# BassyKuo/DAVO

Measured on NVIDIA B200. Metric: PoseNN+attention frame-pairs/sec @128x416, higher is better.
Workload: dtype tf32 operands (activations and weights), fp32 accumulate; inputs read as given (uint8 frames, float32 flow and labels; flow_f16 off)

## Files before the change

davo_b200/_capi.py:

```python
from __future__ import annotations

import ctypes as C
import os

from . import build as _build

_LIB = None

SYMBOLS = (
    "davo_create", "davo_set_weight", "davo_finalize_weights", "davo_forward",
    "davo_forward_host", "davo_get_intermediate", "davo_last_launch_count",
    "davo_last_host_copy_bytes",
    "davo_profile_layers", "davo_debug_set_conv_impl", "davo_forward_pairs", "davo_forward_host_pairs",
    "davo_forward_features", "davo_debug_flows_to_half", "davo_debug_labels_to_bytes", "davo_forward_host_compact", "davo_bind_host_numa",
    "davo_compose_trajectory", "davo_kitti_errors", "davo_decode_jpeg_batch",
    "davo_forward_host_pairs_async", "davo_forward_host_compact_async", "davo_host_wait",
    "davo_comm_unique_id", "davo_comm_create", "davo_comm_world", "davo_allgather_poses",
    "davo_forward_sequence", "davo_forward_sequence_host",
    "davo_odometry_create", "davo_odometry_push", "davo_odometry_reset", "davo_odometry_frames",
    "davo_odometry_push_many", "davo_odometry_push_many_host", "davo_odometry_move",
    "davo_last_error",
    "davo_destroy", "davo_build_info", "davo_config_bytes", "davo_odometry_destroy",
)


class DavoConfigC(C.Structure):
    _fields_ = [(n, C.c_int32) for n in (
        "H", "W", "max_batch", "posenn", "cnv6_out", "in_mode", "att_src", "att_tgt_ones",
        "mask_mode", "se_act", "flow_abs", "flow_norm", "posenn_se", "micro_batch", "depth_norm", "se_pool", "se_hidden",
        "pixel_map", "depth_split", "flow_f16", "batch_norm")]


class DavoFeaturesC(C.Structure):
    _fields_ = [(n, C.c_void_p) for n in (
        "image", "attention", "masked_image", "seg_19", "seg_color", "flow_color", "cnv6_rot", "cnv6_trans")]


def lib_path() -> str:
    return _build.LIB


def load() -> C.CDLL:
    global _LIB
    if _LIB is not None:
        return _LIB
    path = lib_path()
    if _build.is_stale():
        try:
            _build.build()
        except Exception as e:
            if not os.path.exists(path):
                raise ImportError("libdavo_b200.so is not built and cannot be built here: %s" % e)
    try:
        lib = C.CDLL(path)
    except OSError as e:
        raise ImportError("cannot load %s: %s (there is no CPU fallback)" % (path, e))
    for s in SYMBOLS:
        if not hasattr(lib, s):
            raise ImportError("%s does not export %s" % (path, s))
    vp, ip, fp = C.c_void_p, C.c_int, C.POINTER(C.c_float)
    lib.davo_create.argtypes = [C.POINTER(DavoConfigC), ip, C.POINTER(vp)]
    lib.davo_set_weight.argtypes = [vp, C.c_char_p, vp, C.POINTER(C.c_int64), ip]
    lib.davo_finalize_weights.argtypes = [vp]
    lib.davo_forward.argtypes = [vp, ip, vp, vp, vp, vp, vp, vp]
    lib.davo_forward_host.argtypes = [vp, ip, vp, vp, vp, vp, vp, vp]
    lib.davo_forward_pairs.argtypes = [vp, ip, ip, vp, vp, vp, vp, vp, vp]
    lib.davo_forward_host_pairs.argtypes = [vp, ip, ip, vp, vp, vp, vp, vp, vp]
    lib.davo_forward_host_compact.argtypes = [vp, ip, ip, vp, vp, vp, vp, vp, vp]
    lib.davo_bind_host_numa.argtypes = [vp]
    lib.davo_compose_trajectory.argtypes = [vp, vp, ip, vp, vp]
    lib.davo_kitti_errors.argtypes = [vp, vp, vp, ip, vp, fp, vp]
    lib.davo_decode_jpeg_batch.argtypes = [vp, C.POINTER(vp), C.POINTER(C.c_int64), ip, vp, vp]
    lib.davo_forward_host_pairs_async.argtypes = [vp, ip, ip, vp, vp, vp, vp, vp, vp, C.POINTER(C.c_longlong)]
    lib.davo_forward_host_compact_async.argtypes = [vp, ip, ip, vp, vp, vp, vp, vp, vp, C.POINTER(C.c_longlong)]
    lib.davo_host_wait.argtypes = [vp, C.c_longlong]
    lib.davo_forward_sequence.argtypes = [vp, ip, ip, vp, vp, vp, vp, vp, vp, vp]
    lib.davo_forward_sequence_host.argtypes = [vp, ip, ip, vp, vp, vp, vp, vp, vp, vp, C.POINTER(C.c_longlong)]
    lib.davo_odometry_create.argtypes = [vp, ip, ip, ip, C.POINTER(vp)]
    lib.davo_odometry_push.argtypes = [vp, ip, vp, vp, vp, vp, vp, vp, vp, C.POINTER(ip), C.POINTER(ip), vp,
                                       C.POINTER(C.c_longlong)]
    lib.davo_odometry_push_many.argtypes = [ip, C.POINTER(vp), C.POINTER(ip)] + [C.POINTER(vp)] * 7 + [
        C.POINTER(ip), C.POINTER(ip), vp]
    lib.davo_odometry_push_many_host.argtypes = [ip, C.POINTER(vp), C.POINTER(ip)] + [C.POINTER(vp)] * 7 + [
        C.POINTER(ip), C.POINTER(ip), vp, C.POINTER(C.c_longlong)]
    lib.davo_odometry_move.argtypes = [vp, vp]
    lib.davo_odometry_reset.argtypes = [vp]
    lib.davo_odometry_frames.argtypes = [vp, C.POINTER(C.c_longlong), C.POINTER(C.c_longlong)]
    lib.davo_odometry_destroy.argtypes = [vp]
    lib.davo_odometry_destroy.restype = None
    lib.davo_get_intermediate.argtypes = [vp, C.c_char_p, ip, vp, C.c_int64, C.POINTER(C.c_int64)]
    lib.davo_last_launch_count.argtypes = [vp]
    lib.davo_last_host_copy_bytes.argtypes = [vp, C.POINTER(C.c_longlong), C.POINTER(C.c_longlong)]
    lib.davo_profile_layers.argtypes = [vp, ip, fp, C.POINTER(ip), vp]
    lib.davo_debug_set_conv_impl.argtypes = [vp, ip]
    lib.davo_forward_features.argtypes = [vp, ip, vp, vp, vp, vp, vp, C.POINTER(DavoFeaturesC), vp]
    lib.davo_debug_flows_to_half.argtypes = [vp, vp, C.c_longlong, ip]
    lib.davo_debug_labels_to_bytes.argtypes = [vp, vp, C.c_longlong, ip]
    lib.davo_comm_unique_id.argtypes = [vp]
    lib.davo_comm_create.argtypes = [vp, vp, ip, ip]
    lib.davo_comm_world.argtypes = [vp, C.POINTER(ip), C.POINTER(ip)]
    lib.davo_allgather_poses.argtypes = [vp, vp, vp, ip, vp, vp]
    lib.davo_last_error.argtypes = [vp]
    lib.davo_last_error.restype = C.c_char_p
    lib.davo_destroy.argtypes = [vp]
    lib.davo_destroy.restype = None
    lib.davo_build_info.restype = C.c_char_p
    lib.davo_config_bytes.restype = ip
    if lib.davo_config_bytes() != C.sizeof(DavoConfigC):
        raise ImportError("%s: davo_config is %d bytes in the library, %d in this binding (rebuild: python davo_b200/build.py --force)"
                          % (path, lib.davo_config_bytes(), C.sizeof(DavoConfigC)))
    for s in SYMBOLS[:SYMBOLS.index("davo_last_error")]:
        getattr(lib, s).restype = ip
    _LIB = lib
    return lib


PAIRS = {"all": 0, "trajectory": 1, "trajectory_first": 2}


def last_error(lib, handle) -> str:
    msg = lib.davo_last_error(handle)
    return msg.decode() if msg else ""
```

davo_b200/csrc/conv_cm.cuh:

```cuda
#pragma once
#include "conv_common.cuh"

namespace davo {
namespace cm {

constexpr int kBlockM = 128;
constexpr int kThreads = 352;
constexpr int kEpiWarps = 8;
constexpr int kWBytes = kBlockM * kSlabBytes;

struct ConvParams {
  int num_tiles;
  int num_pixel_tiles;
  int tiles_w, tiles_h, groups, m_blocks;
  int Hout, Wout;
  int out_stride;
  int cout_g;
  int cin_group_off;
  int n_patches, n_taps;
  int patch_w;
  int patch_bytes;
  int patch_stage_bytes;
  int p_stages, w_stages;
  int raw;
  float* out;
  const float* bias;
  float* sum_out;
  PatchDesc patches[kMaxPatches];
  TapDesc taps[kMaxTaps];
};

struct TileCoord { int n, g, mb, h0, w0, t; };

template <int NPIX>
__device__ __forceinline__ TileCoord decode_item_cluster(const ConvParams& p, int item, int rank) {
  TileCoord c;
  c.mb = item % p.m_blocks;
  int r = item / p.m_blocks;
  c.g = r % p.groups;
  const int pp = r / p.groups;
  const int tpi = p.tiles_h * p.tiles_w;
  const int pix = min(2 * pp + rank, p.num_pixel_tiles - 1);
  c.t = pix % tpi;
  c.n = pix / tpi;
  c.h0 = (c.t / p.tiles_w) * (NPIX / kTileW);
  c.w0 = (c.t % p.tiles_w) * kTileW;
  return c;
}

template <int NPIX>
__device__ __forceinline__ TileCoord decode_tile(const ConvParams& p, int tile) {
  TileCoord c;
  c.mb = tile % p.m_blocks;
  int r = tile / p.m_blocks;
  const int tpi = p.tiles_h * p.tiles_w;
  c.t = r % tpi;
  r /= tpi;
  c.g = r % p.groups;
  c.n = r / p.groups;
  c.h0 = (c.t / p.tiles_w) * (NPIX / kTileW);
  c.w0 = (c.t % p.tiles_w) * kTileW;
  return c;
}

template <int NPIX, int EPI, bool STAGED = false, bool CLUSTER = false>
__global__ void __launch_bounds__(kThreads, 1)
conv_tc_kernel(const __grid_constant__ CUtensorMap tmX, const __grid_constant__ CUtensorMap tmW,
               const __grid_constant__ CUtensorMap tmO, const __grid_constant__ ConvParams p) {
  extern __shared__ uint8_t smem_raw[];
  uint8_t* smem = reinterpret_cast<uint8_t*>((reinterpret_cast<uintptr_t>(smem_raw) + 1023) &
                                             ~uintptr_t(1023));
  const int PS = p.p_stages, WS = p.w_stages;
  uint8_t* smem_p = smem;
  uint8_t* smem_w = smem + PS * p.patch_stage_bytes;
  uint8_t* epi_stage = smem_w + WS * kWBytes;
  uint64_t* bars = reinterpret_cast<uint64_t*>(epi_stage + (STAGED ? kEpiWarps * 4096 : 0));
  uint64_t* p_full = bars;
  uint64_t* p_empty = bars + kMaxStages;
  uint64_t* w_full = bars + 2 * kMaxStages;
  uint64_t* w_empty = bars + 3 * kMaxStages;
  uint64_t* acc_full = bars + 4 * kMaxStages;
  uint64_t* acc_empty = acc_full + 2;
  uint32_t* tmem_slot = reinterpret_cast<uint32_t*>(acc_empty + 2);
// ... 23 lines not shown
      mbar_init(&w_empty[i], CLUSTER ? 2 : 1);
    }
    for (int i = 0; i < 2; ++i) {
      mbar_init(&acc_full[i], 1);
      mbar_init(&acc_empty[i], EPI == EPI_STORE_RELU ? kEpiWarps : 4);
    }
    fence_mbar_init();
  }
  if (warp == 1) tmem_alloc(tmem_slot, kTmemCols);
  tc_fence_before();
  __syncthreads();
  if constexpr (CLUSTER) cluster_sync();
  tc_fence_after();
  const uint32_t tmem_base = *tmem_slot;

  if (warp == 0) {
    if (lane == 0) {
      pdl_wait();
      int ps = 0;
      uint32_t pphase = 0;
      for (int tile = first; tile < p.num_tiles; tile += step) {
        const TileCoord tc = decode(tile);
        for (int pi = 0; pi < p.n_patches; ++pi) {
          const PatchDesc d = p.patches[pi];
          TWAIT(0, mbar_wait(&p_empty[ps], pphase ^ 1));
          mbar_expect_tx(&p_full[ps], p.patch_bytes);
          tma_load_5d(smem_p + ps * p.patch_stage_bytes, &tmX, &p_full[ps],
                      tc.g * p.cin_group_off + d.c, tc.w0 + d.dw, d.par, tc.h0 + d.dh, tc.n);
          if (++ps == PS) { ps = 0; pphase ^= 1; }
        }
      }
    }
  } else if (warp == 6) {
    if (lane == 0) {
      int ws = 0;
      uint32_t wphase = 0;
      for (int tile = first; tile < p.num_tiles; tile += step) {
        const TileCoord tc = decode(tile);
        const int row0 = (tc.g * p.m_blocks + tc.mb) * p.n_taps;
        for (int t = 0; t < p.n_taps; ++t) {
          TWAIT(1, mbar_wait(&w_empty[ws], wphase ^ 1));
          mbar_expect_tx(&w_full[ws], kWBytes);
          if constexpr (CLUSTER)
            tma_load_2d_multicast(smem_w + ws * kWBytes + rank * (kWBytes / 2), &tmW, &w_full[ws], 0,
                                  (row0 + p.taps[t].b_idx) * kBlockM + rank * (kBlockM / 2), (uint16_t)3);
          else
            tma_load_2d(smem_w + ws * kWBytes, &tmW, &w_full[ws], 0, (row0 + p.taps[t].b_idx) * kBlockM);
          if (++ws == WS) { ws = 0; wphase ^= 1; }
        }
      }
    }
  } else if (warp == 1) {
    {
      constexpr uint32_t idesc = umma_idesc_tf32(kBlockM, NPIX);
      const uint32_t tmem_u = __shfl_sync(0xffffffffu, tmem_base, 0);
      const uint32_t w_hi = umma_desc_hi(1024), x_hi = umma_desc_hi((uint32_t)p.patch_w * kSlabBytes);
      const uint32_t p_lo0 = umma_desc_lo(smem_u32(smem_p)), p_lo_step = (uint32_t)p.patch_stage_bytes >> 4;
      const uint32_t w_lo0 = umma_desc_lo(smem_u32(smem_w));
      int ps = 0, ws = 0;
      uint32_t pphase = 0, wphase = 0;
      int it = 0;
      for (int tile = first; tile < p.num_tiles; tile += step, ++it) {
        const int acc = it & 1;
        const uint32_t acc_phase = (it >> 1) & 1;
        TWAIT(4, mbar_wait(&acc_empty[acc], acc_phase ^ 1));
        tc_fence_after();
        const uint32_t d = tmem_u + acc * NPIX;
        int ti = 0;
        for (int pi = 0; pi < p.n_patches; ++pi) {
          const int nt = p.patches[pi].ntaps;
          TWAIT(2, mbar_wait(&p_full[ps], pphase));
          DAVO_MMA_FENCE();
          const uint32_t pa = p_lo0 + (uint32_t)ps * p_lo_step;
          for (int t = 0; t < nt; ++t, ++ti) {
            const uint32_t x_lo = pa + (uint32_t)p.taps[ti].a_off * (kSlabBytes / 16);
            TWAIT(3, mbar_wait(&w_full[ws], wphase));
            DAVO_MMA_FENCE();
            if (elect_one()) {
              tc_mma_tf32_slab(d, w_lo0 + (uint32_t)ws * (kWBytes / 16), w_hi, x_lo, x_hi, idesc, ti != 0);
              if constexpr (CLUSTER) tc_commit_multicast(&w_empty[ws], (uint16_t)3);
              else tc_commit(&w_empty[ws]);
            }
            if (++ws == WS) { ws = 0; wphase ^= 1; }
          }
          if (elect_one()) tc_commit(&p_empty[ps]);
          if (++ps == PS) { ps = 0; pphase ^= 1; }
        }
        if (elect_one()) tc_commit(&acc_full[acc]);
        __syncwarp();
      }
    }
  } else if (EPI == EPI_STORE_RELU || warp < 6) {
    const int q = warp & 3;
    const int half = warp > 6 ? 1 : 0;
    int it = 0;
    for (int tile = first; tile < p.num_tiles; tile += step, ++it) {
      const int acc = it & 1;
      const uint32_t acc_phase = (it >> 1) & 1;
      const TileCoord tc = decode(tile);
      const int co = tc.mb * kBlockM + q * 32 + lane;
      const bool co_ok = co < p.cout_g;
      const float bias = co_ok ? __ldg(p.bias + tc.g * p.cout_g + co) : 0.f;
      TWAIT(5, mbar_wait(&acc_full[acc], acc_phase));
      tc_fence_after();
#ifdef DAVO_TIMING
      const long long t_busy0 = clock64();
#endif
      const uint32_t t0 = tmem_base + acc * NPIX + (uint32_t(q * 32) << 16);
      const bool warp_has_work = tc.mb * kBlockM + q * 32 < p.cout_g;
      if constexpr (EPI == EPI_STORE_RELU) {
        const size_t pix_stride = p.out_stride;
        float* const obase = p.out + ((size_t)tc.n * p.Hout * p.Wout) * pix_stride + tc.g * p.cout_g + co;
        if constexpr (STAGED) {
          const uint32_t stg = smem_u32(epi_stage) + (half * 4 + q) * 4096;
          uint32_t lane_off[8];
#pragma unroll
          for (int k = 0; k < 8; ++k) lane_off[k] = ((((uint32_t)lane >> 2) ^ k) << 4) | ((lane & 3) << 2);
          if (warp_has_work) {
#pragma unroll 1
            for (int n0 = half * 32; n0 < NPIX; n0 += 64) {
              uint32_t v[32];
              tmem_ld_32x32(t0 + n0, v);
              tmem_ld_wait();
#pragma unroll
              for (int j = 0; j < 32; ++j)
                v[j] = __float_as_uint(epi_out(__uint_as_float(v[j]) + bias, ea));
              if (lane == 0) tma_store_wait_read<0>();
              __syncwarp();
#pragma unroll
              for (int j = 0; j < 32; ++j)
                asm volatile("st.shared.b32 [%0], %1;" ::"r"(stg + j * 128 + lane_off[j & 7]), "r"(v[j]) : "memory");
              fence_proxy_async_smem();
// ... 76 lines not shown
```

davo_b200/csrc/conv_common.cuh:

```cuda
#pragma once
#include "ptx.cuh"

namespace davo {

constexpr int kMaxPatches = 32;
constexpr int kMaxTaps = 144;
constexpr int kTileW = 8;
constexpr int kSlabBytes = 128;
constexpr int kConvThreads = 224;
constexpr int kMaxStages = 8;
constexpr int kSmemBudget = 226 * 1024;
constexpr int kBarrierBytes = 512;

struct PatchDesc {
  int16_t c;
  int8_t dw;
  int8_t par;
  int8_t dh;
  uint8_t ntaps;
  uint16_t tap0;
};
struct TapDesc {
  uint16_t a_off;
  uint16_t b_idx;
  uint8_t n16;
  uint8_t dcol16;
  uint8_t brow8;
  uint8_t fresh;
};

enum { EPI_STORE_RELU = 0, EPI_SUM_RELU = 1 };

struct EpiAct { float lo; uint32_t add, mask; };
__device__ __forceinline__ EpiAct epi_act(int raw) {
  EpiAct a;
  a.lo = raw ? __uint_as_float(0xFF800000u) : 0.f;
  a.add = raw ? 0u : 0x1000u;
  a.mask = raw ? 0xFFFFFFFFu : 0xFFFFE000u;
  return a;
}
__device__ __forceinline__ float epi_out(float x, const EpiAct& a) {
  return __uint_as_float((__float_as_uint(fmaxf(x, a.lo)) + a.add) & a.mask);
}

#if defined(DAVO_MMA_FENCES) && DAVO_MMA_FENCES
#define DAVO_MMA_FENCE() tc_fence_after()
#else
#define DAVO_MMA_FENCE() do { } while (0)
#endif

__device__ __forceinline__ uint64_t umma_desc(uint32_t smem_addr, uint32_t sbo_bytes) {
  return (uint64_t)((smem_addr & 0x3FFFFu) >> 4) | (1ull << 16) | ((uint64_t)(sbo_bytes >> 4) << 32) |
         (1ull << 46) | (2ull << 61);
}

#ifdef DAVO_TIMING
__device__ long long g_conv_timing[148 * 8];
#define TWAIT(slot, stmt) do { long long t_ = clock64(); stmt; tacc[slot] += clock64() - t_; } while (0)
#else
#define TWAIT(slot, stmt) stmt
#endif

}
```

davo_b200/csrc/davo_capi.cu:

```cuda
#include "../../include/davo_b200.h"

#include <cuda.h>
#include <cuda_runtime.h>
#include <atomic>

#include <algorithm>
#include <cmath>
#include <cstdlib>
#include <cstdarg>
#include <cstdio>
#include <cstring>
#include <cctype>
#include <sched.h>
#if defined(__SSE2__)
#include <emmintrin.h>
#endif

#include <condition_variable>
#include <functional>
#include <climits>
#include <map>
#include <set>
#include <mutex>
#include <string>
// ... 463 lines not shown
          const int ch = kk % 16;
          const int tx = 2 * w2 + wp + L.pad_l;
          const int ci = (tx >= 0 && tx < L.k) ? L.pc2w[ch] : -1;
          t.e[kk] = Ent{ty, tx, ci};
        }
        taps.push_back(t);
      }
    } else {
      for (int tx = 0; tx < L.k; ++tx) {
        const int dx = tx * L.dil - L.pad_l;
        const int dw = strided ? floordiv(dx, 2) : dx;
        const int wp = strided ? posmod(dx, 2) : 0;
        for (int sl = 0; sl < L.Cin_g / 32; ++sl) {
          Tap t{par, strided ? wp : (strips ? tx : 0), sl, dh, dw, wp * L.Cin_total + sl * 32, std::vector<Ent>(32)};
          for (int kk = 0; kk < 32; ++kk) t.e[kk] = Ent{ty, tx, sl * 32 + kk};
          taps.push_back(t);
        }
      }
    }
  }
  struct Patch { int par, colkey, slab, c, dh0, dw0, dh1, dw1; std::vector<int> idx; };
  std::vector<Patch> patches;
  for (int i = 0; i < (int)taps.size(); ++i) {
    const Tap& t = taps[i];
    Patch* pp = nullptr;
    for (Patch& q : patches) if (q.par == t.par && q.colkey == t.colkey && q.slab == t.slab) pp = &q;
    if (!pp) { patches.push_back(Patch{t.par, t.colkey, t.slab, t.c, t.dh, t.dw, t.dh, t.dw, {}}); pp = &patches.back(); }
    pp->dh0 = std::min(pp->dh0, t.dh); pp->dh1 = std::max(pp->dh1, t.dh);
    pp->dw0 = std::min(pp->dw0, t.dw); pp->dw1 = std::max(pp->dw1, t.dw);
    pp->idx.push_back(i);
  }
  int Hp = 0, Wp = 0;
  for (const Patch& q : patches) {
    Hp = std::max(Hp, TR + q.dh1 - q.dh0);
    Wp = std::max(Wp, kTileW + q.dw1 - q.dw0);
  }
  const int nt = (int)taps.size(), np = (int)patches.size();
  if (nt > kMaxTaps || np > kMaxPatches)
    return fail(ctx, DAVO_ERR_ARG, "%s: %d taps / %d patches exceed the tables", L.name, nt, np);
  PatchDesc pdesc[kMaxPatches];
  TapDesc tdesc[kMaxTaps];
  memset(pdesc, 0, sizeof pdesc);
  memset(tdesc, 0, sizeof tdesc);
  std::vector<int> order;
  for (int pi = 0; pi < np; ++pi) {
    const Patch& q = patches[pi];
    PatchDesc& d = pdesc[pi];
    d.c = (int16_t)q.c; d.dw = (int8_t)q.dw0; d.par = (int8_t)q.par; d.dh = (int8_t)q.dh0;
    d.ntaps = (uint8_t)q.idx.size(); d.tap0 = (uint16_t)order.size();
    for (int i : q.idx) {
      TapDesc& td = tdesc[order.size()];
      td.a_off = (uint16_t)((taps[i].dh - q.dh0) * Wp + (taps[i].dw - q.dw0));
      td.b_idx = (uint16_t)order.size();
      order.push_back(i);
    }
  }
  const int patch_bytes = Hp * Wp * kSlabBytes;
  const int patch_stage = (patch_bytes + 1023) & ~1023;
  const std::vector<float> wr = round_weights_tf32(L, getw, ctx->compensated_rounding);
  auto wq = [&](int g, int ty, int tx, int ci, int n) {
    return wr[((((size_t)g * L.k + ty) * L.k + tx) * L.Cin_w + ci) * L.BN + n];
  };
  const int MB = L.m_blocks;
  const int rows_per_slab = L.orient == 0 ? L.BN : cm::kBlockM;
  const size_t n_slabs = (size_t)L.groups * (L.orient == 0 ? 1 : MB) * nt;
  std::vector<float> pack(n_slabs * rows_per_slab * 32, 0.f);
  for (int g = 0; g < L.groups; ++g)
    for (int mb = 0; mb < (L.orient == 0 ? 1 : MB); ++mb)
      for (int k = 0; k < nt; ++k)
        for (int m = 0; m < rows_per_slab; ++m) {
          const int n = mb * cm::kBlockM + m;
          if (n >= L.BN) continue;
          const size_t slab = L.orient == 0 ? (size_t)g * nt + k : ((size_t)g * MB + mb) * nt + k;
          for (int kk = 0; kk < 32; ++kk) {
            const Ent& e = taps[order[k]].e[kk];
            if (e.ci >= 0)
              pack[(slab * rows_per_slab + m) * 32 + kk] = wq(g, e.ty, e.tx, e.ci, n);
          }
        }
  if (int rc = dev_alloc(ctx, (void**)&L.d_wpack, pack.size() * 4)) return rc;
  CU_OK(cudaMemcpy(L.d_wpack, pack.data(), pack.size() * 4, cudaMemcpyHostToDevice));
  if (int rc = dev_alloc(ctx, (void**)&L.d_bias, bias_host.size() * 4)) return rc;
  CU_OK(cudaMemcpy(L.d_bias, bias_host.data(), bias_host.size() * 4, cudaMemcpyHostToDevice));
  for (int g = 0; g < L.groups; ++g) {
    std::vector<float> hw((size_t)L.k * L.k * L.Cin_w * L.BN);
    for (int ty = 0; ty < L.k; ++ty)
      for (int tx = 0; tx < L.k; ++tx)
        for (int ci = 0; ci < L.Cin_w; ++ci)
          for (int n = 0; n < L.BN; ++n)
            hw[(((size_t)ty * L.k + tx) * L.Cin_w + ci) * L.BN + n] = wq(g, ty, tx, ci, n);
    if (int rc = dev_alloc(ctx, (void**)&L.d_whwio[g], hw.size() * 4)) return rc;
    CU_OK(cudaMemcpy(L.d_whwio[g], hw.data(), hw.size() * 4, cudaMemcpyHostToDevice));
  }
  int p_stages = 0, w_stages = 0;
  if (L.orient == 0) {
    pm::ConvParams& P = L.prm_pm;
    memset(&P, 0, sizeof P);
    P.tiles_w = L.tiles_w; P.tiles_h = L.tiles_h; P.groups = L.groups;
    P.Hout = L.Hout; P.Wout = L.Wout; P.out_stride = L.out_stride;
    P.cin_group_off = L.cin_shared ? 0 : L.Cin_g;
    P.n_patches = np; P.n_taps = nt; P.patch_w = Wp;
    P.patch_bytes = patch_bytes; P.patch_stage_bytes = patch_stage;
    P.bias = L.d_bias;
    memcpy(P.patches, pdesc, sizeof pdesc);
    memcpy(P.taps, tdesc, sizeof tdesc);
    const int bbytes = L.BN * kSlabBytes;
    const int fixed = 1024  + kBarrierBytes + pm::kBiasSmemBytes + pm::kEpiStageBytes;
    const int avail = kSmemBudget - fixed;
    const int resident_bytes = L.groups * nt * bbytes;
    L.b_resident = L.groups == 1 && resident_bytes + 2 * patch_stage <= avail && resident_bytes <= 100 * 1024;
    if (L.b_resident) {
      P.p_stages = std::min(kMaxStages, (avail - resident_bytes) / patch_stage);
      P.b_stages = 0;
      L.smem_bytes = fixed + resident_bytes + P.p_stages * patch_stage;
    } else {
      P.p_stages = 3;
      if ((avail - 3 * patch_stage) / bbytes < 4) P.p_stages = 2;
      P.b_stages = std::min(kMaxStages, (avail - P.p_stages * patch_stage) / bbytes);
      if (P.b_stages < 2) return fail(ctx, DAVO_ERR_ARG, "%s: shared-memory plan does not fit", L.name);
      L.smem_bytes = fixed + P.b_stages * bbytes + P.p_stages * patch_stage;
    }
    p_stages = P.p_stages; w_stages = P.b_stages;
  } else {
    cm::ConvParams& P = L.prm_cm;
    memset(&P, 0, sizeof P);
    P.tiles_w = L.tiles_w; P.tiles_h = L.tiles_h; P.groups = L.groups; P.m_blocks = MB;
    P.Hout = L.Hout; P.Wout = L.Wout; P.out_stride = L.out_stride; P.cout_g = L.BN;
    P.cin_group_off = L.cin_shared ? 0 : L.Cin_g;
    P.n_patches = np; P.n_taps = nt; P.patch_w = Wp;
    P.patch_bytes = patch_bytes; P.patch_stage_bytes = patch_stage;
    P.bias = L.d_bias;
    memcpy(P.patches, pdesc, sizeof pdesc);
    memcpy(P.taps, tdesc, sizeof tdesc);
    const char* stg_env = getenv("DAVO_B200_CM_STAGED");
    L.cm_staged = L.epi == EPI_STORE_RELU && (stg_env ? !strcmp(stg_env, "1") : nt <= 18);
    const int fixed = 1024  + kBarrierBytes + (L.cm_staged ? cm::kEpiWarps * 4096 : 0);
    const int avail = kSmemBudget - fixed;
    P.p_stages = patch_stage <= 40 * 1024 ? 3 : 2;
    if (const char* e = getenv("DAVO_B200_CM_PSTAGES")) P.p_stages = std::max(2, atoi(e));
    if (!getenv("DAVO_B200_CM_PSTAGES") && P.p_stages == 2 && (avail - 3 * patch_stage) / cm::kWBytes >= 5) P.p_stages = 3;
    if (P.p_stages >= 3 && (avail - P.p_stages * patch_stage) / cm::kWBytes < 4) P.p_stages = 2;
    P.w_stages = std::min(kMaxStages, (avail - P.p_stages * patch_stage) / cm::kWBytes);
    if (P.w_stages < 2) return fail(ctx, DAVO_ERR_ARG, "%s: shared-memory plan does not fit", L.name);
    L.smem_bytes = fixed + P.w_stages * cm::kWBytes + P.p_stages * patch_stage;
    p_stages = P.p_stages; w_stages = P.w_stages;
  }
  if (p_stages < 2) return fail(ctx, DAVO_ERR_ARG, "%s: patch ring does not fit", L.name);
  EncodeTiledFn enc = get_encode_fn();
  if (!enc) return fail(ctx, DAVO_ERR_CUDA, "cuTensorMapEncodeTiled entry point not found");
  {
    const cuuint64_t C = L.Cin_total, H = L.Hin, W = L.Win, Hq = L.Hin_p, Wq = L.Win_p, N = ctx->mb;
    cuuint64_t dims[5], strides[4];
    if (strided) {
      dims[0] = 2 * C; dims[1] = Wq / 2; dims[2] = 2; dims[3] = Hq / 2; dims[4] = N;
      strides[0] = 2 * C * 4; strides[1] = Wq * C * 4; strides[2] = 2 * Wq * C * 4; strides[3] = Hq * Wq * C * 4;
    } else {
      dims[0] = C; dims[1] = W; dims[2] = 1; dims[3] = H; dims[4] = N;
      strides[0] = C * 4; strides[1] = Wq * C * 4; strides[2] = Wq * C * 4; strides[3] = Hq * Wq * C * 4;
    }
    const cuuint32_t box[5] = {32, (cuuint32_t)Wp, 1, (cuuint32_t)Hp, 1};
    const cuuint32_t es[5] = {1, 1, 1, 1, 1};
    CUresult r = enc(&L.tmA, CU_TENSOR_MAP_DATA_TYPE_FLOAT32, 5, L.d_in, dims, strides, box, es,
                     CU_TENSOR_MAP_INTERLEAVE_NONE, CU_TENSOR_MAP_SWIZZLE_128B,
                     CU_TENSOR_MAP_L2_PROMOTION_L2_256B, CU_TENSOR_MAP_FLOAT_OOB_FILL_NONE);
    if (r != CUDA_SUCCESS) return fail(ctx, DAVO_ERR_CUDA, "%s: cuTensorMapEncodeTiled(activation) -> %d", L.name, (int)r);
  }
  {
    cuuint64_t dims[2] = {32, (cuuint64_t)n_slabs * rows_per_slab};
    cuuint64_t strides[1] = {128};
    const cuuint32_t box[2] = {32, (cuuint32_t)rows_per_slab};
    const cuuint32_t es[2] = {1, 1};
    CUresult r = enc(&L.tmB, CU_TENSOR_MAP_DATA_TYPE_FLOAT32, 2, L.d_wpack, dims, strides, box, es,
                     CU_TENSOR_MAP_INTERLEAVE_NONE, CU_TENSOR_MAP_SWIZZLE_128B,
                     CU_TENSOR_MAP_L2_PROMOTION_L2_256B, CU_TENSOR_MAP_FLOAT_OOB_FILL_NONE);
    if (r != CUDA_SUCCESS) return fail(ctx, DAVO_ERR_CUDA, "%s: cuTensorMapEncodeTiled(weights) -> %d", L.name, (int)r);
    L.tmB64 = L.tmB;
    const char* cl_env = getenv("DAVO_B200_CLUSTER");
    L.cm_cluster = L.orient == 1 && (L.epi == EPI_STORE_RELU || getenv("DAVO_B200_CNV7_CM")) && !(cl_env && !strcmp(cl_env, "0"));
    if (L.cm_cluster) {
      const cuuint32_t box64[2] = {32, (cuuint32_t)(rows_per_slab / 2)};
      r = enc(&L.tmB64, CU_TENSOR_MAP_DATA_TYPE_FLOAT32, 2, L.d_wpack, dims, strides, box64, es,
              CU_TENSOR_MAP_INTERLEAVE_NONE, CU_TENSOR_MAP_SWIZZLE_128B,
              CU_TENSOR_MAP_L2_PROMOTION_L2_256B, CU_TENSOR_MAP_FLOAT_OOB_FILL_NONE);
      if (r != CUDA_SUCCESS) return fail(ctx, DAVO_ERR_CUDA, "%s: cuTensorMapEncodeTiled(weights, half slab) -> %d", L.name, (int)r);
    }
  }
  L.tmO = L.tmA;
  if (L.pitched_out() && L.epi == EPI_STORE_RELU && !(L.orient == 0 && L.BN >= 32))
    return fail(ctx, DAVO_ERR_ARG, "%s: an odd-sized output map needs the TMA-store epilogue (pixels-on-M, >= 32 channels)", L.name);
  if ((L.orient == 1 && L.cm_staged) || (L.orient == 0 && L.epi == EPI_STORE_RELU && L.BN >= 32))
    if (int rc = encode_output_map(ctx, L, L.out_stride, L.Wout, kTileW)) return rc;
  if (getenv("DAVO_B200_VERBOSE"))
    fprintf(stderr, "[davo_b200] %s: %s, tile %dx8 px, %d m-block(s), patch %dx%d (%d B) x%d, %d taps, weights %s, rings P%d W%d, smem %d\n",
            L.name, L.orient == 0 ? "pixels-on-M" : "channels-on-M", TR, MB, Hp, Wp, patch_bytes, np, nt,
            L.b_resident ? "resident" : "streamed", p_stages, w_stages, L.smem_bytes);
  return 0;
}

template <class GetW>
int plan_layer_wide(davo_ctx* ctx, Layer& L, GetW getw, const std::vector<float>& bias_host) {
  const int G = L.wide_G, TWc = L.wide_tw, THr = 128 / TWc, Co = L.BN, NW = G * Co;
  if (NW != 128) return fail(ctx, DAVO_ERR_ARG, "%s: the widened kernel is built for N = 128 (got %d)", L.name, NW);
  const int C = L.Cin_total, S = 32 / C, half = S / 2, slabs_per_run = 2 * G / S;
  const int d_min = -floordiv(L.pad_l + S - 1, 2), d_max = floordiv(L.k - 1 - L.pad_l, 2), nd = d_max - d_min + 1;
  const int c_min = floordiv(-L.pad_l, S), c_max = floordiv(2 * (G - 1) + L.k - 1 - L.pad_l, S);
  const std::vector<float> wr = round_weights_tf32(L, getw, ctx->compensated_rounding);
  auto wq = [&](int ty, int tx, int ci, int n) { return wr[(((size_t)ty * L.k + tx) * L.Cin_w + ci) * Co + n]; };
  const int box_rows = nd * Co;
  std::vector<float> pack((size_t)L.k * box_rows * 32, 0.f);
  for (int ty = 0; ty < L.k; ++ty)
    for (int b = 0; b < nd; ++b)
      for (int n = 0; n < Co; ++n)
        for (int kk = 0; kk < 32; ++kk) {
          const int tx = 2 * (d_max - b) + kk / C + L.pad_l, ci = L.pc2w[kk % C];
          if (tx >= 0 && tx < L.k && ci >= 0) pack[(((size_t)ty * nd + b) * Co + n) * 32 + kk] = wq(ty, tx, ci, n);
        }
  if (int rc = dev_alloc(ctx, (void**)&L.d_wpack, pack.size() * 4)) return rc;
  CU_OK(cudaMemcpy(L.d_wpack, pack.data(), pack.size() * 4, cudaMemcpyHostToDevice));
  std::vector<float> bias_rep((size_t)NW);
  for (int i = 0; i < NW; ++i) bias_rep[i] = bias_host[i % Co];
  if (int rc = dev_alloc(ctx, (void**)&L.d_bias, bias_rep.size() * 4)) return rc;
  CU_OK(cudaMemcpy(L.d_bias, bias_rep.data(), bias_rep.size() * 4, cudaMemcpyHostToDevice));
  {
    std::vector<float> hw((size_t)L.k * L.k * L.Cin_w * Co);
    for (int ty = 0; ty < L.k; ++ty)
      for (int tx = 0; tx < L.k; ++tx)
        for (int ci = 0; ci < L.Cin_w; ++ci)
          for (int n = 0; n < Co; ++n) hw[(((size_t)ty * L.k + tx) * L.Cin_w + ci) * Co + n] = wq(ty, tx, ci, n);
    if (int rc = dev_alloc(ctx, (void**)&L.d_whwio[0], hw.size() * 4)) return rc;
    CU_OK(cudaMemcpy(L.d_whwio[0], hw.data(), hw.size() * 4, cudaMemcpyHostToDevice));
  }
  auto g_lo_of = [&](int c) { return std::max(half * c - d_max, 0); };
  auto g_hi_of = [&](int c) { return std::min(half * c - d_min, G - 1); };
  struct Cover { int c, from; };
  std::vector<Cover> cover;
  for (int s0 = 0; s0 < G;) {
    int best = c_min - 1;
    for (int c = c_min; c <= c_max; ++c)
      if (g_lo_of(c) <= s0 && s0 <= g_hi_of(c) && (best < c_min || g_hi_of(c) > g_hi_of(best))) best = c;
    if (best < c_min) return fail(ctx, DAVO_ERR_ARG, "%s: widened plan cannot cover the run", L.name);
    cover.push_back(Cover{best, s0});
    s0 = g_hi_of(best) + 1;
  }
  const int par0 = posmod(-L.pad_t, 2);
  struct P2 { int c, par, from; };
  std::vector<P2> plist;
  for (const Cover& cv : cover) plist.push_back(P2{cv.c, par0, cv.from});
  for (int par = 0; par < 2; ++par)
// ... 2137 lines not shown
    if (cap < nbr * 256) return too_small(nbr * 256);
    for (int br = 0; br < nbr; ++br)
      for (int ch = 0; ch < 256; ++ch) {
        float a = 0.f;
        for (int i = 0; i < np; ++i) a += tmp[((size_t)br * np + i) * 256 + ch];
        out[br * 256 + ch] = a;
      }
    *n_out = nbr * 256;
    return 0;
  } else if (li >= 0) {
    const Layer& L = ctx->layers[li];
    const bool rep6 = li == 5 && c.posenn_se == 3;
    if (part.empty() || part == "pitched") {
      if (!L.d_out) return fail(ctx, DAVO_ERR_ARG, "davo_get_intermediate: %s is not stored by this variant", L.name);
      const int64_t per = (int64_t)L.Hout_p * L.Wout_p * L.out_stride;
      if (part == "pitched" || !L.pitched_out()) { n = per; src = L.d_out + (size_t)pair * per; }
      else {
        n = (int64_t)L.Hout * L.Wout * L.out_stride;
        if (cap < n) return too_small(n);
        const size_t row = (size_t)L.Wout * L.out_stride * 4;
        CU_OK(cudaMemcpy2D(out, row, L.d_out + (size_t)pair * per, (size_t)L.Wout_p * L.out_stride * 4, row, L.Hout, cudaMemcpyDeviceToHost));
        *n_out = n;
        return 0;
      }
    } else if (part == "in") {
      if (rep6) return fail(ctx, DAVO_ERR_ARG, "davo_get_intermediate: %s is not computed by this variant", L.name);
      n = (int64_t)L.Hin_p * L.Win_p * L.Cin_total; src = L.d_in + (size_t)pair * n;
      if (li == 0)
        if (int rc = materialise_packed()) return rc;
    } else if (part == "b") {
      if (rep6) return fail(ctx, DAVO_ERR_ARG, "davo_get_intermediate: %s is not computed by this variant", L.name);
      n = (int64_t)L.groups * L.BN; src = c.batch_norm ? L.d_beta : L.d_bias;
    } else if (part.size() >= 2 && part[0] == 'w' && part.find_first_not_of("0123456789", 1) == std::string::npos) {
      const int g = atoi(part.c_str() + 1);
      if (rep6) return fail(ctx, DAVO_ERR_ARG, "davo_get_intermediate: %s is not computed by this variant", L.name);
      if (g >= L.groups) return fail(ctx, DAVO_ERR_ARG, "davo_get_intermediate: %s has %d group(s)", L.name, L.groups);
      const int T = L.k * L.k;
      n = (int64_t)T * L.Cin_g * L.BN;
      if (cap < n) return too_small(n);
      std::vector<float> hw((size_t)T * L.Cin_w * L.BN);
      CU_OK(cudaMemcpy(hw.data(), L.d_whwio[g], hw.size() * 4, cudaMemcpyDeviceToHost));
      for (int t = 0; t < T; ++t)
        for (int j = 0; j < L.Cin_g; ++j) {
          const int ci = li == 0 ? L.pc2w[j] : j;
          for (int o = 0; o < L.BN; ++o) out[((size_t)t * L.Cin_g + j) * L.BN + o] = ci >= 0 ? hw[((size_t)t * L.Cin_w + ci) * L.BN + o] : 0.f;
        }
      *n_out = n;
      return 0;
    } else if (part == "plan") {
      if (rep6) return fail(ctx, DAVO_ERR_ARG, "davo_get_intermediate: %s is not computed by this variant", L.name);
      const Layer& P = pick_layer(ctx, (size_t)li, ctx->last_npairs_mb);
      const float v[] = {(float)P.orient, (float)P.npix, (float)P.wide_G, (float)P.wide_tw, (float)P.cm_staged,
                         (float)P.cm_cluster, (float)P.strips, (float)P.m_blocks, (float)P.groups, (float)(c.batch_norm ? 1 : 0),
                         (float)P.epi, (float)P.BN, (float)P.b_resident, (float)P.fused_front};
      n = (int64_t)(sizeof v / sizeof v[0]);
      if (cap < n) return too_small(n);
      for (int i = 0; i < n; ++i) out[i] = v[i];
      *n_out = n;
      return 0;
    }
  }
  if (!src) return fail(ctx, DAVO_ERR_ARG, "davo_get_intermediate: unknown name '%s'", name);
  if (cap < n) return too_small(n);
  CU_OK(cudaMemcpy(out, src, (size_t)n * 4, cudaMemcpyDeviceToHost));
  *n_out = n;
  return 0;
}

#ifdef DAVO_TIMING
extern "C" int davo_debug_layer_timing(davo_ctx* ctx, int layer, long long* out, void* stream) {
  if (!ctx || layer < 0 || layer > 6 || !out) return DAVO_ERR_ARG;
  cudaStream_t st = reinterpret_cast<cudaStream_t>(stream);
  const int npairs = std::min(ctx->last_B * (ctx->unit_sample ? 1 : 2), ctx->mb);
  Layer& L = pick_layer(ctx, (size_t)layer, npairs);
  if (int rc = launch_conv(ctx, L, npairs, st)) return rc;
  if (int rc = launch_conv(ctx, L, npairs, st)) return rc;
  CU_OK(cudaStreamSynchronize(st));
  CU_OK(cudaMemcpyFromSymbol(out, davo::g_conv_timing, sizeof(long long) * 148 * 8));
  return 0;
}
#endif

extern "C" int davo_debug_set_conv_impl(davo_ctx* ctx, int impl) {
  if (!ctx || impl < 0 || impl > 1) return DAVO_ERR_ARG;
  ctx->conv_impl = impl;
  return 0;
}

extern "C" int davo_profile_layers(davo_ctx* ctx, int iters, float* ms_out, int* npairs_out,
                                   void* stream) {
  if (!ctx || !ms_out || iters <= 0) return DAVO_ERR_ARG;
  if (!ctx->finalized || ctx->last_npairs_mb == 0) return fail(ctx, DAVO_ERR_STATE, "davo_profile_layers: run a forward first");
  CU_OK(cudaSetDevice(ctx->device));
  cudaStream_t st = reinterpret_cast<cudaStream_t>(stream);
  const int npairs = std::min(ctx->last_B * (ctx->unit_sample ? 1 : 2), ctx->mb);
  if (npairs_out) *npairs_out = npairs;
  cudaEvent_t e0, e1;
  CU_OK(cudaEventCreate(&e0));
  CU_OK(cudaEventCreate(&e1));
  int dummy = 0;
  auto timed = [&](auto&& fn, float* ms_dst) -> int {
    if (int rc = fn()) return rc;
    CU_OK(cudaEventRecord(e0, st));
    for (int it = 0; it < iters; ++it)
      if (int rc = fn()) return rc;
    CU_OK(cudaEventRecord(e1, st));
    CU_OK(cudaEventSynchronize(e1));
// ... 205 lines not shown
  float* stats = reinterpret_cast<float*>(base + off_stats);
  kitti_dist_kernel<<<1, 32, 0, st>>>(reinterpret_cast<const Mat4*>(gt), n, dist);
  kitti_segments_kernel<<<(count + 127) / 128, 128, 0, st>>>(reinterpret_cast<const Mat4*>(gt), reinterpret_cast<const Mat4*>(res), dist, n, n_first, segs);
  kitti_stats_kernel<<<1, 32, 0, st>>>(segs, count, stats);
  CU_OK(cudaGetLastError());
  CU_OK(cudaMemcpyAsync(stats_host, stats, 3 * sizeof(float), cudaMemcpyDeviceToHost, st));
  CU_OK(cudaStreamSynchronize(st));
  return 0;
}

extern "C" int davo_decode_jpeg_batch(davo_ctx* ctx, const uint8_t* const* jpeg, const int64_t* nbytes, int n, uint8_t* img_dev,
                                      void* stream) {
  if (!ctx) return DAVO_ERR_ARG;
  if (!jpeg || !nbytes || !img_dev || n < 1) return fail(ctx, DAVO_ERR_ARG, "davo_decode_jpeg_batch: null buffer or no images");
  const davo_jpeg::Api& j = davo_jpeg::api();
  if (!j.why.empty()) return fail(ctx, DAVO_ERR_STATE, "davo_decode_jpeg_batch: %s", j.why.c_str());
  CU_OK(cudaSetDevice(ctx->device));
  cudaStream_t st = reinterpret_cast<cudaStream_t>(stream);
  if (!ctx->jpeg_handle) {
    if (j.CreateSimple(&ctx->jpeg_handle) != NVJPEG_STATUS_SUCCESS) return fail(ctx, DAVO_ERR_CUDA, "nvjpegCreateSimple failed");
    if (j.StateCreate(ctx->jpeg_handle, &ctx->jpeg_state) != NVJPEG_STATUS_SUCCESS) return fail(ctx, DAVO_ERR_CUDA, "nvjpegJpegStateCreate failed");
  }
  const int H = ctx->cfg.H, W3 = 3 * ctx->cfg.W;
  for (int i = 0; i < n; ++i) {
    int comps = 0, ws[NVJPEG_MAX_COMPONENT], hs[NVJPEG_MAX_COMPONENT];
    nvjpegChromaSubsampling_t sub;
    if (j.GetImageInfo(ctx->jpeg_handle, jpeg[i], (size_t)nbytes[i], &comps, &sub, ws, hs) != NVJPEG_STATUS_SUCCESS)
      return fail(ctx, DAVO_ERR_ARG, "davo_decode_jpeg_batch: image %d is not a JPEG nvJPEG can parse", i);
    if (ws[0] != W3 || hs[0] != H)
      return fail(ctx, DAVO_ERR_ARG, "davo_decode_jpeg_batch: image %d is %dx%d, the frame triple must be %dx%d", i, hs[0], ws[0], H, W3);
    nvjpegImage_t out;
    memset(&out, 0, sizeof out);
    out.channel[0] = img_dev + (size_t)i * H * W3 * 3;
    out.pitch[0] = (size_t)W3 * 3;
    const nvjpegStatus_t rc = j.Decode(ctx->jpeg_handle, ctx->jpeg_state, jpeg[i], (size_t)nbytes[i], NVJPEG_OUTPUT_RGBI, &out, st);
    if (rc != NVJPEG_STATUS_SUCCESS) return fail(ctx, DAVO_ERR_CUDA, "nvjpegDecode(image %d) -> %d", i, (int)rc);
  }
  CU_OK(cudaStreamSynchronize(st));
  return 0;
}

extern "C" int davo_debug_labels_to_bytes(const float* src, uint8_t* dst, long long n, int portable) {
  if (!src || !dst || n < 0) return DAVO_ERR_ARG;
  if (portable) davo_host::labels_to_bytes_portable(src, dst, (size_t)n);
  else davo_host::labels_to_bytes(src, dst, (size_t)n);
  return 0;
}

extern "C" int davo_debug_flows_to_half(const float* src, uint16_t* dst, long long n, int portable) {
  if (!src || !dst || n < 0) return DAVO_ERR_ARG;
  const bool ok = portable ? davo_host::flows_to_half_portable(src, dst, (size_t)n) : davo_host::flows_to_half(src, dst, (size_t)n);
  return ok ? 0 : 1;
}
```

include/davo_b200.h:

```cpp
#ifndef DAVO_B200_H
#define DAVO_B200_H

#include <stdint.h>

#ifdef __cplusplus
extern "C" {
#endif

typedef struct davo_ctx davo_ctx;

enum davo_status {
  DAVO_OK = 0,
  DAVO_ERR_ARG = -1,
  DAVO_ERR_CUDA = -2,
  DAVO_ERR_WEIGHT = -3,
  DAVO_ERR_STATE = -4
};

typedef struct davo_config {
  int32_t H, W;
  int32_t max_batch;
  int32_t posenn;
  int32_t cnv6_out;
  int32_t in_mode;
// ... 56 lines not shown
                      void* cuda_stream);

int davo_forward_host_compact(davo_ctx*, int B, int pairs, const uint8_t* img_u8, const uint16_t* flow_f16,
                              const uint8_t* seg_u8, const float* depth, float* pose_out, void* cuda_stream);

int davo_forward_host_pairs_async(davo_ctx*, int B, int pairs, const uint8_t* img_u8, const float* flow,
                                  const float* seg, const float* depth, float* pose_out, void* cuda_stream,
                                  long long* ticket);
int davo_forward_host_compact_async(davo_ctx*, int B, int pairs, const uint8_t* img_u8, const uint16_t* flow_f16,
                                    const uint8_t* seg_u8, const float* depth, float* pose_out, void* cuda_stream,
                                    long long* ticket);
int davo_host_wait(davo_ctx*, long long ticket);

int davo_forward_sequence(davo_ctx*, int n_frames, int pairs, const uint8_t* img_u8, const float* flow_fwd,
                          const float* flow_bwd, const float* seg, const float* depth, float* pose_out,
                          void* cuda_stream);
int davo_forward_sequence_host(davo_ctx*, int n_frames, int pairs, const uint8_t* img_u8, const float* flow_fwd,
                               const float* flow_bwd, const float* seg, const float* depth, float* pose_out,
                               void* cuda_stream, long long* ticket);

typedef struct davo_odometry davo_odometry;
int davo_odometry_create(davo_ctx*, int max_push, int pairs, int host_inputs, davo_odometry** out);
int davo_odometry_push(davo_odometry*, int k, const uint8_t* img, const float* flow_fwd, const float* flow_bwd,
                       const float* seg, const float* depth, float* pose_out, double* traj_out, int* n_samples,
                       int* n_traj, void* cuda_stream, long long* ticket);
int davo_odometry_push_many(int n, davo_odometry* const* sessions, const int* k, const uint8_t* const* img,
                            const float* const* flow_fwd, const float* const* flow_bwd, const float* const* seg,
                            const float* const* depth, float* const* pose_out, double* const* traj_out,
                            int* n_samples, int* n_traj, void* cuda_stream);
int davo_odometry_push_many_host(int n, davo_odometry* const* sessions, const int* k, const uint8_t* const* img,
                                 const float* const* flow_fwd, const float* const* flow_bwd, const float* const* seg,
                                 const float* const* depth, float* const* pose_out, double* const* traj_out,
                                 int* n_samples, int* n_traj, void* cuda_stream, long long* ticket);
int davo_odometry_reset(davo_odometry*);
int davo_odometry_frames(const davo_odometry*, long long* pushed, long long* posed);
void davo_odometry_destroy(davo_odometry*);
int davo_odometry_move(davo_odometry*, davo_ctx* dst);

int davo_bind_host_numa(davo_ctx*);

int davo_get_intermediate(davo_ctx*, const char* name, int pair, float* out,
                          int64_t cap, int64_t* n);

int davo_last_host_copy_bytes(const davo_ctx*, long long* h2d, long long* d2h);

int davo_last_launch_count(const davo_ctx*);

int davo_profile_layers(davo_ctx*, int iters, float* ms_out, int* npairs_out,
                        void* cuda_stream);

int davo_debug_set_conv_impl(davo_ctx*, int impl);
int davo_debug_flows_to_half(const float* src, uint16_t* dst, long long n, int portable);
int davo_debug_labels_to_bytes(const float* src, uint8_t* dst, long long n, int portable);

#define DAVO_COMM_ID_BYTES 128
int davo_comm_unique_id(void* id128);
int davo_comm_create(davo_ctx*, const void* id128, int rank, int world);
int davo_comm_world(const davo_ctx*, int* rank, int* world);
int davo_allgather_poses(davo_ctx*, void* nccl_comm, const float* local_dev, int n_local,
                         float* all_dev, void* cuda_stream);

typedef struct davo_kitti_segment {
  int32_t first_frame, last_frame;
  float r_err, t_err, len, speed;
} davo_kitti_segment;
int davo_compose_trajectory(davo_ctx*, const float* poses_dev, int n_samples, double* traj_dev, void* cuda_stream);
int davo_kitti_errors(davo_ctx*, const double* gt_dev, const double* res_dev, int n_frames,
                      davo_kitti_segment* seg_dev, float* stats_host, void* cuda_stream);

int davo_decode_jpeg_batch(davo_ctx*, const uint8_t* const* jpeg, const int64_t* nbytes, int n, uint8_t* img_dev,
                           void* cuda_stream);

const char* davo_last_error(const davo_ctx*);
void davo_destroy(davo_ctx*);
const char* davo_build_info(void);
int davo_config_bytes(void);

#ifdef __cplusplus
}
#endif
#endif
```

Measured before the change: 97090.

## Skip MMA rows that read only zero padding in channels-on-M convs

For channels-on-M convolution tiles, each tap's MMA is narrowed to the output rows whose shifted input lies inside the feature map, and the MMA is skipped entirely when no rows are valid. The first tap still runs over the full tile so the accumulator is initialised. This removes tensor-core work on border tiles that would only multiply zero padding. It adds per-tap index arithmetic in the MMA-issue warp. Correctness depends on the TMA map bounds now being expressed as map_h/map_w. It is enabled by default for 256-pixel tiles and can be turned off with an environment variable.

```diff
diff --git a/davo_b200/_capi.py b/davo_b200/_capi.py
--- a/davo_b200/_capi.py
+++ b/davo_b200/_capi.py
@@ -13,6 +13,7 @@
     "davo_last_host_copy_bytes",
     "davo_profile_layers", "davo_debug_set_conv_impl", "davo_forward_pairs", "davo_forward_host_pairs",
     "davo_forward_features", "davo_debug_flows_to_half", "davo_debug_labels_to_bytes", "davo_forward_host_compact", "davo_bind_host_numa",
+    "davo_debug_mma_rows_in_map",
     "davo_compose_trajectory", "davo_kitti_errors", "davo_decode_jpeg_batch",
     "davo_forward_host_pairs_async", "davo_forward_host_compact_async", "davo_host_wait",
     "davo_comm_unique_id", "davo_comm_create", "davo_comm_world", "davo_allgather_poses",
@@ -96,6 +97,7 @@
     lib.davo_forward_features.argtypes = [vp, ip, vp, vp, vp, vp, vp, C.POINTER(DavoFeaturesC), vp]
     lib.davo_debug_flows_to_half.argtypes = [vp, vp, C.c_longlong, ip]
     lib.davo_debug_labels_to_bytes.argtypes = [vp, vp, C.c_longlong, ip]
+    lib.davo_debug_mma_rows_in_map.argtypes = [ip] * 7 + [C.POINTER(ip)] * 2
     lib.davo_comm_unique_id.argtypes = [vp]
     lib.davo_comm_create.argtypes = [vp, vp, ip, ip]
     lib.davo_comm_world.argtypes = [vp, C.POINTER(ip), C.POINTER(ip)]
diff --git a/davo_b200/csrc/conv_cm.cuh b/davo_b200/csrc/conv_cm.cuh
--- a/davo_b200/csrc/conv_cm.cuh
+++ b/davo_b200/csrc/conv_cm.cuh
@@ -23,12 +23,15 @@
   int patch_stage_bytes;
   int p_stages, w_stages;
   int raw;
+  int pad_skip;
+  int map_h, map_w;
   float* out;
   const float* bias;
   float* sum_out;
   PatchDesc patches[kMaxPatches];
   TapDesc taps[kMaxTaps];
 };
+static_assert(sizeof(ConvParams) <= 4096, "kernel parameter block");
 
 struct TileCoord { int n, g, mb, h0, w0, t; };
 
@@ -158,7 +161,8 @@
     }
   } else if (warp == 1) {
     {
-      constexpr uint32_t idesc = umma_idesc_tf32(kBlockM, NPIX);
+      constexpr int TR = NPIX / kTileW;
+      constexpr uint32_t idesc_n0 = umma_idesc_tf32(kBlockM, 0);
       const uint32_t tmem_u = __shfl_sync(0xffffffffu, tmem_base, 0);
       const uint32_t w_hi = umma_desc_hi(1024), x_hi = umma_desc_hi((uint32_t)p.patch_w * kSlabBytes);
       const uint32_t p_lo0 = umma_desc_lo(smem_u32(smem_p)), p_lo_step = (uint32_t)p.patch_stage_bytes >> 4;
@@ -172,6 +176,7 @@
         TWAIT(4, mbar_wait(&acc_empty[acc], acc_phase ^ 1));
         tc_fence_after();
         const uint32_t d = tmem_u + acc * NPIX;
+        const TileCoord tc = decode(tile);
         int ti = 0;
         for (int pi = 0; pi < p.n_patches; ++pi) {
           const int nt = p.patches[pi].ntaps;
@@ -179,11 +184,18 @@
           DAVO_MMA_FENCE();
           const uint32_t pa = p_lo0 + (uint32_t)ps * p_lo_step;
           for (int t = 0; t < nt; ++t, ++ti) {
-            const uint32_t x_lo = pa + (uint32_t)p.taps[ti].a_off * (kSlabBytes / 16);
+            const TapDesc td = p.taps[ti];
+            MmaRows w{0, TR};
+            if (p.pad_skip && ti != 0) w = mma_rows_in_map(p.map_h, p.map_w, tc.h0, tc.w0, TR, td.dy, td.dx);
+            const uint32_t x_lo = pa + ((uint32_t)td.a_off + (uint32_t)(w.r_lo * p.patch_w)) * (kSlabBytes / 16);
+            const uint32_t idesc = idesc_n0 | ((uint32_t)(w.r_hi - w.r_lo) << 17);
+            const bool issue = w.r_hi > w.r_lo;
             TWAIT(3, mbar_wait(&w_full[ws], wphase));
             DAVO_MMA_FENCE();
             if (elect_one()) {
-              tc_mma_tf32_slab(d, w_lo0 + (uint32_t)ws * (kWBytes / 16), w_hi, x_lo, x_hi, idesc, ti != 0);
+              if (issue)
+                tc_mma_tf32_slab(d + (uint32_t)(w.r_lo * kTileW), w_lo0 + (uint32_t)ws * (kWBytes / 16), w_hi, x_lo,
+                                 x_hi, idesc, ti != 0);
               if constexpr (CLUSTER) tc_commit_multicast(&w_empty[ws], (uint16_t)3);
               else tc_commit(&w_empty[ws]);
             }
diff --git a/davo_b200/csrc/conv_common.cuh b/davo_b200/csrc/conv_common.cuh
--- a/davo_b200/csrc/conv_common.cuh
+++ b/davo_b200/csrc/conv_common.cuh
@@ -27,7 +27,18 @@
   uint8_t dcol16;
   uint8_t brow8;
   uint8_t fresh;
+  int8_t dy, dx;
 };
+
+struct MmaRows { int r_lo, r_hi; };
+__host__ __device__ __forceinline__ MmaRows mma_rows_in_map(int Hext, int Wext, int h0, int w0, int TR, int dy, int dx) {
+  const int y0 = h0 + dy, x0 = w0 + dx;
+  int lo = min(max(-y0, 0), TR), hi = min(max(Hext - y0, 0), TR);
+  if (lo >= hi || x0 + kTileW <= 0 || x0 >= Wext) return MmaRows{0, 0};
+  lo &= ~1;
+  hi += hi & 1;
+  return MmaRows{lo, hi};
+}
 
 enum { EPI_STORE_RELU = 0, EPI_SUM_RELU = 1 };
 
diff --git a/davo_b200/csrc/davo_capi.cu b/davo_b200/csrc/davo_capi.cu
--- a/davo_b200/csrc/davo_capi.cu
+++ b/davo_b200/csrc/davo_capi.cu
@@ -539,6 +539,7 @@
       TapDesc& td = tdesc[order.size()];
       td.a_off = (uint16_t)((taps[i].dh - q.dh0) * Wp + (taps[i].dw - q.dw0));
       td.b_idx = (uint16_t)order.size();
+      td.dy = (int8_t)taps[i].dh; td.dx = (int8_t)taps[i].dw;
       order.push_back(i);
     }
   }
@@ -579,6 +580,7 @@
     if (int rc = dev_alloc(ctx, (void**)&L.d_whwio[g], hw.size() * 4)) return rc;
     CU_OK(cudaMemcpy(L.d_whwio[g], hw.data(), hw.size() * 4, cudaMemcpyHostToDevice));
   }
+  const int map_h = strided ? L.Hin_p / 2 : L.Hin, map_w = strided ? L.Win_p / 2 : L.Win;
   int p_stages = 0, w_stages = 0;
   if (L.orient == 0) {
     pm::ConvParams& P = L.prm_pm;
@@ -619,6 +621,9 @@
     P.bias = L.d_bias;
     memcpy(P.patches, pdesc, sizeof pdesc);
     memcpy(P.taps, tdesc, sizeof tdesc);
+    const char* skip_env = getenv("DAVO_B200_PAD_SKIP");
+    P.pad_skip = !(skip_env && !strcmp(skip_env, "0")) && L.npix == 256;
+    P.map_h = map_h; P.map_w = map_w;
     const char* stg_env = getenv("DAVO_B200_CM_STAGED");
     L.cm_staged = L.epi == EPI_STORE_RELU && (stg_env ? !strcmp(stg_env, "1") : nt <= 18);
     const int fixed = 1024  + kBarrierBytes + (L.cm_staged ? cm::kEpiWarps * 4096 : 0);
@@ -636,13 +641,13 @@
   EncodeTiledFn enc = get_encode_fn();
   if (!enc) return fail(ctx, DAVO_ERR_CUDA, "cuTensorMapEncodeTiled entry point not found");
   {
-    const cuuint64_t C = L.Cin_total, H = L.Hin, W = L.Win, Hq = L.Hin_p, Wq = L.Win_p, N = ctx->mb;
+    const cuuint64_t C = L.Cin_total, Hq = L.Hin_p, Wq = L.Win_p, N = ctx->mb;
     cuuint64_t dims[5], strides[4];
     if (strided) {
-      dims[0] = 2 * C; dims[1] = Wq / 2; dims[2] = 2; dims[3] = Hq / 2; dims[4] = N;
+      dims[0] = 2 * C; dims[1] = map_w; dims[2] = 2; dims[3] = map_h; dims[4] = N;
       strides[0] = 2 * C * 4; strides[1] = Wq * C * 4; strides[2] = 2 * Wq * C * 4; strides[3] = Hq * Wq * C * 4;
     } else {
-      dims[0] = C; dims[1] = W; dims[2] = 1; dims[3] = H; dims[4] = N;
+      dims[0] = C; dims[1] = map_w; dims[2] = 1; dims[3] = map_h; dims[4] = N;
       strides[0] = C * 4; strides[1] = Wq * C * 4; strides[2] = Wq * C * 4; strides[3] = Hq * Wq * C * 4;
     }
     const cuuint32_t box[5] = {32, (cuuint32_t)Wp, 1, (cuuint32_t)Hp, 1};
@@ -677,10 +682,26 @@
     return fail(ctx, DAVO_ERR_ARG, "%s: an odd-sized output map needs the TMA-store epilogue (pixels-on-M, >= 32 channels)", L.name);
   if ((L.orient == 1 && L.cm_staged) || (L.orient == 0 && L.epi == EPI_STORE_RELU && L.BN >= 32))
     if (int rc = encode_output_map(ctx, L, L.out_stride, L.Wout, kTileW)) return rc;
-  if (getenv("DAVO_B200_VERBOSE"))
+  if (getenv("DAVO_B200_VERBOSE")) {
     fprintf(stderr, "[davo_b200] %s: %s, tile %dx8 px, %d m-block(s), patch %dx%d (%d B) x%d, %d taps, weights %s, rings P%d W%d, smem %d\n",
             L.name, L.orient == 0 ? "pixels-on-M" : "channels-on-M", TR, MB, Hp, Wp, patch_bytes, np, nt,
             L.b_resident ? "resident" : "streamed", p_stages, w_stages, L.smem_bytes);
+    if (L.orient == 1) {
+      auto cyc = [](int rows) { return rows ? 4.0 * std::max(53.8, 8.0 * rows / 2) : 0.0; };
+      double full = 0, skipped = 0;
+      for (int th = 0; th < L.tiles_h; ++th)
+        for (int tw = 0; tw < L.tiles_w; ++tw)
+          for (int t = 0; t < nt; ++t) {
+            const MmaRows w = mma_rows_in_map(map_h, map_w, th * TR, tw * kTileW, TR, tdesc[t].dy, tdesc[t].dx);
+            full += cyc(TR);
+            if (t != 0) skipped += cyc(TR) - cyc(w.r_hi - w.r_lo);
+          }
+      const double scale = (double)L.groups * MB * ctx->mb;
+      fprintf(stderr, "[davo_b200] %s: padding skip %s: %.1f of %.1f M MMA cycles per pass of %d pairs on padding only (%.1f %%)\n",
+              L.name, L.prm_cm.pad_skip ? "on" : "off", skipped * scale * 1e-6, full * scale * 1e-6, ctx->mb,
+              100.0 * skipped / full);
+    }
+  }
   return 0;
 }
 
@@ -2924,7 +2945,8 @@
       const Layer& P = pick_layer(ctx, (size_t)li, ctx->last_npairs_mb);
       const float v[] = {(float)P.orient, (float)P.npix, (float)P.wide_G, (float)P.wide_tw, (float)P.cm_staged,
                          (float)P.cm_cluster, (float)P.strips, (float)P.m_blocks, (float)P.groups, (float)(c.batch_norm ? 1 : 0),
-                         (float)P.epi, (float)P.BN, (float)P.b_resident, (float)P.fused_front};
+                         (float)P.epi, (float)P.BN, (float)P.b_resident, (float)P.fused_front,
+                         (float)(P.orient == 1 ? P.prm_cm.pad_skip : 0)};
       n = (int64_t)(sizeof v / sizeof v[0]);
       if (cap < n) return too_small(n);
       for (int i = 0; i < n; ++i) out[i] = v[i];
@@ -3236,3 +3258,12 @@
   const bool ok = portable ? davo_host::flows_to_half_portable(src, dst, (size_t)n) : davo_host::flows_to_half(src, dst, (size_t)n);
   return ok ? 0 : 1;
 }
+
+extern "C" int davo_debug_mma_rows_in_map(int map_h, int map_w, int h0, int w0, int tile_rows, int dy, int dx,
+                                          int* r_lo, int* r_hi) {
+  if (!r_lo || !r_hi || (tile_rows != 16 && tile_rows != 32)) return DAVO_ERR_ARG;
+  const MmaRows w = mma_rows_in_map(map_h, map_w, h0, w0, tile_rows, dy, dx);
+  *r_lo = w.r_lo;
+  *r_hi = w.r_hi;
+  return 0;
+}
diff --git a/include/davo_b200.h b/include/davo_b200.h
--- a/include/davo_b200.h
+++ b/include/davo_b200.h
@@ -132,6 +132,8 @@
 int davo_debug_set_conv_impl(davo_ctx*, int impl);
 int davo_debug_flows_to_half(const float* src, uint16_t* dst, long long n, int portable);
 int davo_debug_labels_to_bytes(const float* src, uint8_t* dst, long long n, int portable);
+int davo_debug_mma_rows_in_map(int map_h, int map_w, int h0, int w0, int tile_rows, int dy, int dx,
+                               int* r_lo, int* r_hi);
 
 #define DAVO_COMM_ID_BYTES 128
 int davo_comm_unique_id(void* id128);
```

Result: no change. 97660 (median of 6 runs) (+0.6%).
